# kestrelquantum/QuantumCollocation.jl

Hardware: AMD Instinct MI355X
Metric: full-trajectory constraint+Jacobian evals/s, 3-qubit T=1000 (higher is better)
Workload: dtype f64; 1 GPU; 3-qubit Toffoli UnitarySmoothPulseProblem, T=1000; T=1000 knots (1000/GPU), Pade order 4, free dt; T=1000, N=8, n_drives=6, kernel=mfma, parallelism=knot-shard x1, output_ring_buffers=17

## Files before the change

### quantumcollocation.jl_amd/csrc/qc_mfma_kernels.hip

```cpp
#include "qc_mfma_common.h"

namespace {

using namespace qc_mfma;

constexpr int kIntervalsPerWG = 1;
constexpr int kThreads = 128 * kIntervalsPerWG;
constexpr int kMaxGrid = 1024;

__device__ inline v4d load_GA(const double* __restrict__ Gx, int mat, int lane) { return load_image_tile(Gx + mat * 256, lane); }

constexpr int kDF = QC_DWIN_MAX_DERIV;


template <int kMU>
__device__ inline void request_images(int m, const double* __restrict__ Gx, int lane, v4d& g0, v4d (&gk)[kMU]) {
    g0 = load_GA(Gx, 0, lane);
#pragma unroll
    for (int u = 0; u < kMU; ++u) {
        const int k = u < m ? u : (m > 0 ? m - 1 : 0);
        gk[u] = load_GA(Gx, m > 0 ? k + 1 : 0, lane);
    }
}
template <int kMU>
__device__ inline void assemble_G_request(const QcParams& P, const double* __restrict__ Gx, const double* __restrict__ z0, int lane,
                                          v4d& g0, v4d (&gk)[kMU], double& av) {
    av = load_amp_lanes(z0, P.off_a, P.m, lane);
    request_images(P.m, Gx, lane, g0, gk);
}
template <int kMU>
__device__ inline v4d assemble_G_combine(const QcParams& P, const double* __restrict__ Gx, int lane, const v4d& g0, const v4d (&gk)[kMU],
                                         double av, double (&ak)[kMU]) {
    const int m = P.m;
    v4d Ga = g0;
#pragma unroll
    for (int u = 0; u < kMU; ++u) {
        ak[u] = (u < m) ? bcast_lane(av, u) : 0.0;
        Ga += ak[u] * gk[u];
    }
    for (int k = kMU; k < m; ++k) Ga += bcast_lane(av, k) * load_GA(Gx, k + 1, lane);
    return Ga;
}
template <int kMU>
__device__ inline v4d assemble_G(const QcParams& P, const double* __restrict__ Gx, const double* __restrict__ z0,
                                 int lane, v4d (&gk)[kMU], double (&ak)[kMU]) {
    v4d g0;
    double av;
    assemble_G_request(P, Gx, z0, lane, g0, gk, av);
    return assemble_G_combine(P, Gx, lane, g0, gk, av, ak);
}

template <int MODE>
__device__ inline void store_tile_T(double* __restrict__ p, const v4d& x, int g, int j) {
#pragma unroll
    for (int r = 0; r < 4; ++r) qc_st8m<MODE>(p + (4 * r + g) * 16 + j, x[r]);
}

template <int MODE>
__device__ inline void store_tile_T_masked(double* __restrict__ p, const v4d& x, int nr, int g, int j) {
#pragma unroll
    for (int r = 0; r < 4; ++r) if (4 * r + g < nr && j < nr) qc_st8m<MODE>(p + (4 * r + g) * nr + j, x[r]);
}
template <bool MASK>
__device__ inline v4d load_state_tile(const double* __restrict__ zU, int col, int nr, int g) {
    if constexpr (!MASK) {
        const double* p = zU + col * 16 + g;
        return v4d{p[0], p[4], p[8], p[12]};
    } else {
        const double* p = zU + col * nr;
        v4d v;
#pragma unroll
        for (int r = 0; r < 4; ++r) v[r] = (4 * r + g < nr) ? p[4 * r + g] : 0.0;
        return v;
    }
}

constexpr int kLdsGa = 0, kLdsU0 = 256, kLdsU1 = 512, kLdsGk = 768;

__device__ inline void lds_put(double* __restrict__ base, int lane, const v4d& x) {
    v2d* p = reinterpret_cast<v2d*>(base) + lane;
    p[0] = v2d{x[0], x[1]};
    p[64] = v2d{x[2], x[3]};
}
__device__ inline v4d lds_get(const double* __restrict__ base, int lane) {
    const v2d* p = reinterpret_cast<const v2d*>(base) + lane;
    const v2d lo = p[0], hi = p[64];
    return v4d{lo[0], lo[1], hi[0], hi[1]};
}
__device__ inline v2d load_knot128(const double* __restrict__ p, int lane) {
    typedef v2d __attribute__((aligned(8))) v2d_u;
    return reinterpret_cast<const v2d_u*>(p)[lane];
}
__device__ inline v4d lds_state_tile(const double* __restrict__ U, int col, int g) {
    const double* p = U + col * 16 + g;
    return v4d{p[0], p[4], p[8], p[12]};
}

#define QC_HOT_ARGS(P) (P).Gx, dZ, (P).t_begin, (P).n_int, (P).zdim, (P).off_a, (P).off_dt, (P).m

template <bool JAC, int MODE, bool DIAG, int kMU, bool KET, bool BATCH, bool ONCE = false, bool HEAD = false>
__global__ __launch_bounds__(JAC ? kThreads : 64, 2) void qc_mfma16_pade4_kernel(const double* __restrict__ hot_Gx, const double* __restrict__ Z, long long hot_t_begin, int hot_n_int,
                                                                      int hot_zdim, int hot_off_a, int hot_off_dt, int hot_m, const QcParams Pk,
                                                                      double* __restrict__ F, double* __restrict__ J,
                                                                      const QcParams* __restrict__ Pb) {
    const QcParams& P = BATCH ? Pb[blockIdx.y] : Pk;
    const int h_n_int = BATCH ? P.n_int : hot_n_int, h_zdim = BATCH ? P.zdim : hot_zdim, h_off_a = BATCH ? P.off_a : hot_off_a;
    const int h_off_dt = BATCH ? P.off_dt : hot_off_dt;
    const long long h_t_begin = BATCH ? P.t_begin : hot_t_begin;
    constexpr int kLdsD0 = kLdsGk + kMU * 256, kLdsD1 = kLdsD0 + 128;
    constexpr int kLdsBlock = kLdsD1 + 128;
    static_assert((kMU / 2 + 1) * 272 <= kLdsD0, "the windows must lie beyond the compute wave's transpose scratch");
    __shared__ __attribute__((aligned(16))) double sm_all[JAC ? kIntervalsPerWG * kLdsBlock : 2];
    unsigned long long t_entry = 0, t_kernarg = 0;
    if constexpr (DIAG) {
        t_entry = __builtin_amdgcn_s_memrealtime();
        const long long dep = (long long)Pk.N + Pk.n_deriv + Pk.drow[7] + Pk.jac_nnz + Pk.jo_d + Pk.ho_d + (long long)Pk.G + (long long)Pk.stamps +
                              (long long)Z + (long long)Pb + (long long)(Pk.c[2] != 0.0) + (long long)(Pk.dt_fixed != 0.0);
        asm volatile("s_memrealtime %0" : "=s"(t_kernarg) : "s"(dep));
    }
#ifndef QC_NO_KERNARG_TOUCH
    QcKernargTouch<sizeof(QcParams) + 96> touch;
    touch.request();
#endif
    const int tid = threadIdx.x;
    const int lane0 = tid & 63;
    const int wave = JAC ? __builtin_amdgcn_readfirstlane(tid >> 6) : 0;
    const int role = JAC ? 1 - wave / kIntervalsPerWG : 0;
    const int slot = wave % kIntervalsPerWG;
    double* __restrict__ sm = sm_all + (JAC ? slot * kLdsBlock : 0);
    const int ipw = JAC ? kIntervalsPerWG : 1;
    const int n_wg = (h_n_int + ipw - 1) / ipw;
    static_assert(!HEAD || (JAC && ONCE && !KET && !BATCH), "HEAD is a form of the loop-free unitary F + dF instantiation");
    const int m = HEAD ? kMU : BATCH ? P.m : hot_m;
    const int nc = KET ? P.nc : 8;
    const int nr = KET ? P.n : 16;
    const bool ft = HEAD || h_off_dt >= 0;
    const double c1 = P.c[1], c2 = P.c[2];
    const double* __restrict__ Gx = BATCH ? P.Gx : hot_Gx;

    v4d g0_img, gk_img[kMU];
    if (JAC && role == 1) request_images(m, Gx, lane0, g0_img, gk_img);
#ifndef QC_NO_KERNARG_TOUCH
    touch.consume();
#endif
    int vb = blockIdx.x;
    if (vb >= n_wg) return;
    do {
        int lane = lane0;
        if constexpr (!ONCE) asm volatile("" : "+v"(lane));
        const int g = lane >> 4, j = lane & 15, jj = j & 7;
        const int jc = (!KET || jj < nc) ? jj : 0;
        const bool left = j < 8;
        const v4d IdB = identity_B(g, j);
        const int b_raw = qc_xcd_remap(vb, n_wg) * ipw + slot;
        const bool active = b_raw < h_n_int;
        const int b = active ? b_raw : h_n_int - 1;
        const long long t = h_t_begin + b;
        const double* __restrict__ z0 = Z + t * (long long)h_zdim;
        const double* __restrict__ z1 = z0 + h_zdim;
        const double av_pre = (JAC && role == 1) ? load_amp_lanes(z0, h_off_a, m, lane) : 0.0;
        const double h_pre = ft ? load_uniform(z0 + h_off_dt) : opaque_scalar(P.dt_fixed);
        double* __restrict__ Jb = JAC ? J + (size_t)b * P.J_stride + P.J_off : nullptr;
        double* __restrict__ Fb = (HEAD || F) ? F + (size_t)b * P.F_stride + P.F_off : nullptr;
        QC_STAMP_DECL;

        if (HEAD ? __builtin_expect(role == 1, 1) : (JAC && role == 1)) {
            if (!active) { __syncthreads(); if constexpr (!ONCE) __syncthreads(); continue; }
            __builtin_amdgcn_s_setprio(3);
            if constexpr (DIAG) {
                qc_ts_[9] = t_entry;
                if (!(P.dbg_skip & 4)) { qc_ts_[10] = t_kernarg; qc_ts_[11] = __builtin_amdgcn_s_getreg((4 << 0) | (0 << 6) | (31 << 11)) | (1ull << 40); }
            }
            QC_STAMP(P, b, lane, 0);
            const double h = h_pre;
            double ak[kMU];
            const double av = av_pre;
            const v4d& g0 = g0_img;
            const v4d (&gk)[kMU] = gk_img;
            v4d u0, u1;
            v2d w_u0, w_u1;
            if constexpr (KET) {
                u0 = load_state_tile<true>(z0 + P.off_U, jc, nr, g);
                u1 = load_state_tile<true>(z1 + P.off_U, jc, nr, g);
            } else {
                w_u0 = load_knot128(z0 + P.off_U, lane);
                w_u1 = load_knot128(z1 + P.off_U, lane);
            }
            const int wo = P.dwin_lo + (2 * lane < P.dwin_n ? 2 * lane : 0);
            const v2d w_d0 = load_knot128(z0 + wo, 0), w_d1 = load_knot128(z1 + wo, 0);
            if (DIAG && (P.dbg_skip & 4)) {
                asm volatile("s_waitcnt lgkmcnt(0)" ::: "memory");
                QC_STAMP(P, b, lane, 10);
                asm volatile("s_waitcnt vmcnt(0)" ::: "memory");
                QC_STAMP(P, b, lane, 11);
            }
            v4d Ga;
            if constexpr (HEAD) {
                Ga = g0;
#pragma unroll
                for (int u = 0; u < kMU; ++u) Ga += bcast_lane(av, u) * gk[u];
            } else {
                Ga = assemble_G_combine(P, Gx, lane, g0, gk, av, ak);
            }
            const double hc1 = h * c1, hc2 = h * h * c2;
            QC_STAMP(P, b, lane, 1);
            bool skip = false;
            if constexpr (DIAG) skip = (P.dbg_skip & 1) != 0;
            const v4d Gb = mm16(Ga, IdB);
            const v4d G2T = mm16(Gb, Ga);
            v4d Fm, Bm;
#pragma unroll
            for (int r = 0; r < 4; ++r) {
                const double ev = IdB[r] + hc2 * G2T[r];
                Fm[r] = -(ev + hc1 * Ga[r]);
                Bm[r] = ev - hc1 * Ga[r];
            }
#ifndef QC_EARLY_COPIES
#define QC_EARLY_COPIES 4
#endif
            constexpr int kEarly = (!KET && ONCE) ? QC_EARLY_COPIES : 0;
            auto early_copy = [&](int q) {
                store_tile_T<MODE>(Jb + P.jo_F + q * 256, Fm, g, j);
                store_tile_T<MODE>(Jb + P.jo_B + q * 256, Bm, g, j);
            };
            auto hand_off = [&]() {
                lds_put(sm + kLdsGa, lane, Ga);
                if constexpr (KET) {
                    lds_put(sm + kLdsU0, lane, u0);
                    lds_put(sm + kLdsU1, lane, u1);
                } else {
                    reinterpret_cast<v2d*>(sm + kLdsU0)[lane] = w_u0;
                    reinterpret_cast<v2d*>(sm + kLdsU1)[lane] = w_u1;
                }
                reinterpret_cast<v2d*>(sm + kLdsD0)[lane] = w_d0;
                reinterpret_cast<v2d*>(sm + kLdsD1)[lane] = w_d1;
#pragma unroll
                for (int u = 0; u < kMU; ++u)
                    if (u < m) lds_put(sm + kLdsGk + u * 256, lane, gk[u]);
            };
            if constexpr (kEarly > 0) {
                if (HEAD || (!skip && P.copies >= kEarly)) {
#pragma unroll
                    for (int q = 0; q < kEarly; ++q) early_copy(q);
                    hand_off();
                } else {
                    if (!skip)
                        for (int q = 0; q < P.copies; ++q) early_copy(q);
                    hand_off();
                }
            } else {
                hand_off();
            }
            __syncthreads();
            if (!skip) {
                double* pF = Jb + P.jo_F;
                double* pB = Jb + P.jo_B;
                const int ncop = HEAD ? 8 : P.copies;
                for (int q = kEarly; q < ncop; ++q) {
                    if constexpr (!KET) {
                        store_tile_T<MODE>(pF + q * 256, Fm, g, j);
                        store_tile_T<MODE>(pB + q * 256, Bm, g, j);
                    } else {
                        store_tile_T_masked<MODE>(pF + q * nr * nr, Fm, nr, g, j);
                        store_tile_T_masked<MODE>(pB + q * nr * nr, Bm, nr, g, j);
                    }
                }
                __builtin_amdgcn_s_setprio(0);
                QC_STAMP(P, b, lane, 2);
                {
                    if (HEAD || P.dwin_n > 0) {
                        const double* w0 = sm + kLdsD0 - P.dwin_lo;
                        const double* w1 = sm + kLdsD1 - P.dwin_lo;
                        int jo = P.jo_d;
#pragma unroll
                        for (int d = 0; d < kDF; ++d) {
                            if (d < P.n_deriv) {
                                const int dim = P.ddim_i[d], r0 = P.drow[d];
                                if (lane < dim) {
                                    const double dxv = w0[P.dx_off[d] + lane];
                                    const double dfv = w1[P.x_off[d] + lane] - w0[P.x_off[d] + lane];
                                    if (Fb) Fb[r0 + lane] = dfv - h * dxv;
                                    Jb[jo + lane] = -1.0;
                                    Jb[jo + dim + lane] = 1.0;
                                    Jb[jo + 2 * dim + lane] = -h;
                                    if (ft) Jb[jo + 3 * dim + lane] = -dxv;
                                }
                                jo += (ft ? 4 : 3) * dim;
                            }
                        }
                    } else {
                        deriv_rows_generic(P, z0, z1, h, Fb, Jb, lane, false);
                    }
                }
                if constexpr (DIAG) {
                    asm volatile("s_waitcnt vmcnt(0)" ::: "memory");
                    QC_STAMP(P, b, lane, 3);
                }
                QC_STAMP_FLUSH(P, b, lane, 0, 3);
                QC_STAMP_FLUSH(P, b, lane, 9, 11);
            }
            if constexpr (!ONCE) __syncthreads();
            continue;
        }

        if (!active) { if constexpr (JAC) { __syncthreads(); if constexpr (!ONCE) __syncthreads(); } continue; }
        __builtin_amdgcn_s_setprio(1);
        QC_STAMP(P, b, lane, 4);
        QC_STAMP_CYCLES(13);
        const double h = h_pre;
        v4d u0, u1, Ga;
        v4d gk[kMU];
        if constexpr (JAC) {
            __syncthreads();
            Ga = lds_get(sm + kLdsGa, lane);
            if constexpr (KET) {
                u0 = lds_get(sm + kLdsU0, lane);
                u1 = lds_get(sm + kLdsU1, lane);
            } else {
                u0 = lds_state_tile(sm + kLdsU0, jc, g);
                u1 = lds_state_tile(sm + kLdsU1, jc, g);
            }
        } else {
            u0 = load_state_tile<KET>(z0 + P.off_U, jc, nr, g);
            u1 = load_state_tile<KET>(z1 + P.off_U, jc, nr, g);
            double ak[kMU];
            Ga = assemble_G(P, Gx, z0, lane, gk, ak);
        }
        const double hc1 = h * c1, hc2 = h * h * c2;
        QC_STAMP(P, b, lane, 5);
        bool skipc = false;
        if constexpr (DIAG) skipc = (P.dbg_skip & 2) != 0;
        if (!skipc) {
            v4d W, Wsw;
#pragma unroll
            for (int r = 0; r < 4; ++r) {
                const double sm_ = u1[r] + u0[r], df = u1[r] - u0[r];
                W[r] = left ? sm_ : df;
                Wsw[r] = left ? df : sm_;
            }
            const v4d P1 = mm16(Ga, W);
            const v4d P1sw = swap8(P1);
            v4d Q;
#pragma unroll
            for (int r = 0; r < 4; ++r) Q[r] = left ? (-hc1 * W[r] + hc2 * P1sw[r]) : (hc2 * W[r]);
            constexpr int NB = JAC ? kMU + 1 : 1;
            v4d sB[NB];
            {
                v4d aB[NB], bB[NB];
                aB[0] = Ga;
                bB[0] = P1sw;
                if constexpr (JAC) {
#pragma unroll
                    for (int u = 0; u < kMU; ++u) {
                        aB[u + 1] = lds_get(sm + kLdsGk + (u < m ? u : m - 1) * 256, lane);
                        bB[u + 1] = Q;
                    }
                }
                mm16_multi<NB>(aB, bB, sB);
            }
            const v4d P2 = sB[0];
            QC_STAMP(P, b, lane, 6);
            v4d E;
            {
                v4d dl, dh;
                const double d1 = -c1, d2 = 2.0 * c2 * h;
#pragma unroll
                for (int r = 0; r < 4; ++r) {
                    dl[r] = Wsw[r] - hc1 * P1[r] + hc2 * P2[r];
                    dh[r] = d1 * P1[r] + d2 * P2[r];
                }
                const v4d dhs = swap8(dh);
#pragma unroll
                for (int r = 0; r < 4; ++r) E[r] = left ? dl[r] : dhs[r];
            }
            constexpr int NC = JAC ? kMU / 2 + 1 : 1;
            v4d sC[NC];
            v4d Y[NC];
            {
                v4d aC[NC], bC[NC];
                aC[0] = E;
                bC[0] = IdB;
                if constexpr (JAC) {
#pragma unroll
                    for (int p2 = 0; p2 < kMU / 2; ++p2) {
                        const v4d R1 = sB[2 * p2 + 1], R2 = sB[2 * p2 + 2];
                        const v4d R1sw = swap8(R1), R2sw = swap8(R2);
                        aC[p2 + 1] = Ga;
#pragma unroll
                        for (int r = 0; r < 4; ++r) {
                            bC[p2 + 1][r] = left ? R1sw[r] : R2[r];
                            Y[p2 + 1][r] = left ? R1[r] : R2sw[r];
                        }
                    }
                }
                if constexpr (JAC) {
                    if constexpr (kMU / 2 > 0) {
                        v4d aT[kMU / 2], bT[kMU / 2], dT[kMU / 2];
#pragma unroll
                        for (int p2 = 0; p2 < kMU / 2; ++p2) { aT[p2] = aC[p2 + 1]; bT[p2] = bC[p2 + 1]; }
                        mm16_multi<kMU / 2>(aT, bT, dT);
#pragma unroll
                        for (int p2 = 0; p2 < kMU / 2; ++p2) sC[p2 + 1] = dT[p2];
                    }
                } else {
                    mm16_multi<NC>(aC, bC, sC);
                }
            }
            v4d ET;
            v4d YT[kMU / 2 > 0 ? kMU / 2 : 1];
            if constexpr (JAC) {
                v4d tin[kMU / 2 + 1], tout[kMU / 2 + 1];
                tin[0] = E;
#pragma unroll
                for (int p2 = 0; p2 < kMU / 2; ++p2) tin[p2 + 1] = Y[p2 + 1] + sC[p2 + 1];
                lds_transpose16_multi<kMU / 2 + 1>(sm, tin, tout, g, j);
                ET = tout[0];
#pragma unroll
                for (int p2 = 0; p2 < kMU / 2; ++p2) YT[p2] = tout[p2 + 1];
            } else {
                ET = sC[0];
            }
            auto store_ET = [&]() {
#pragma unroll
                for (int r = 0; r < 4; ++r) {
                    const int c = 4 * r + g;
                    if (c < 8) {
                        if (Fb && (!KET || (c < nc && j < nr))) qc_st8m<MODE>(Fb + c * nr + j, ET[r]);
                    } else if (JAC && ft && (!KET || (c - 8 < nc && j < nr))) {
                        qc_st8m<MODE>(Jb + P.jo_h + (c - 8) * nr + j, ET[r]);
                    }
                }
            };
            QC_STAMP(P, b, lane, 7);
            if constexpr (!JAC) {
                store_ET();
                deriv_rows_generic(P, z0, z1, h, Fb, nullptr, lane, false);
            } else {
                double* pa = Jb + P.jo_a;
                auto store_pair = [&](int k, const v4d& YTk) {
                    const bool two = k + 1 < m;
                    const int sk = KET ? P.s : 128;
                    double* p = pa + (size_t)k * sk;
#pragma unroll
                    for (int r = 0; r < 4; ++r) {
                        const int c = 4 * r + g;
                        if (r < 2) { if (!KET || (c < nc && j < nr)) qc_st8m<MODE>(p + c * nr + j, YTk[r]); }
                        else if (two && (!KET || (c - 8 < nc && j < nr))) qc_st8m<MODE>(p + sk + (c - 8) * nr + j, YTk[r]);
                    }
                };
                QC_STAMP(P, b, lane, 8);
                store_ET();
#pragma unroll
                for (int u = 0; u < kMU; u += 2)
                    if (u < m) store_pair(u, YT[u >> 1]);
                for (int k = kMU; k < m; k += 2) {
                    const v4d R1 = mm16(load_GA(Gx, k + 1, lane), Q);
                    const v4d R2 = mm16(load_GA(Gx, k + 2 <= m ? k + 2 : k + 1, lane), Q);
                    const v4d R1sw = swap8(R1), R2sw = swap8(R2);
                    v4d X, Yk;
#pragma unroll
                    for (int r = 0; r < 4; ++r) {
                        X[r] = left ? R1sw[r] : R2[r];
                        Yk[r] = left ? R1[r] : R2sw[r];
                    }
                    Yk += mm16(Ga, X);
                    store_pair(k, mm16(Yk, IdB));
                }
            }
            if constexpr (DIAG) {
                asm volatile("s_waitcnt vmcnt(0)" ::: "memory");
                QC_STAMP(P, b, lane, 12);
                QC_STAMP_CYCLES(14);
            }
            if constexpr (DIAG) qc_ts_[15] = __builtin_amdgcn_s_getreg((4 << 0) | (0 << 6) | (31 << 11)) | (1ull << 40);
            QC_STAMP_FLUSH(P, b, lane, 4, 8);
            QC_STAMP_FLUSH(P, b, lane, 12, 15);
        }
        if constexpr (JAC && !ONCE) __syncthreads();
    } while (!ONCE && (vb += gridDim.x) < n_wg);
}

}

bool qc_mfma_pade4_supported(const QcParams& P) {
    return P.integrator == QC_PADE && P.p == 2 && ((P.n <= 16 && P.nc <= 8) || (P.n <= 32 && P.nc <= 16)) && P.m <= 32;
}

size_t qc_mfma_gx_doubles(const QcParams& P) {
    if (P.n > 32) return qc_mfma64_gx_doubles(P);
    return P.n > 16 ? qc_mfma32_gx_doubles(P) : (size_t)2 * (P.m + 1) * 256;
}

void qc_mfma_pack_G(const QcParams& P, const double* G, double* Gx) {
    if (P.n > 32) { qc_mfma64_pack_G(P, G, Gx); return; }
    if (P.n > 16) { qc_mfma32_pack_G(P, G, Gx); return; }
    const int n = P.n, M = P.m + 1;
    for (int mat = 0; mat < M; ++mat) {
        const double* A = G + (size_t)mat * n * n;
        for (int pr = 0; pr < 2; ++pr)
            for (int l = 0; l < 64; ++l)
                for (int e = 0; e < 2; ++e) {
                    const int g = l >> 4, i = l & 15, kk = 2 * pr + e, c = 4 * kk + g;
                    const bool in = i < n && c < n;
                    Gx[((size_t)mat * 2 + pr) * 128 + l * 2 + e] = in ? A[(size_t)c * n + i] : 0.0;
                    Gx[((size_t)(M + mat) * 2 + pr) * 128 + l * 2 + e] = in ? A[(size_t)i * n + c] : 0.0;
                }
    }
}

template <bool JAC, bool DIAG, int MU>
static void launch16m(const QcParams& P, const double* dZ, double* dF, double* dJ, hipStream_t st, int grid, int threads) {
    if (P.nc != 8 || P.n != 16) {
        const int n_wg_k = JAC ? (P.n_int + kIntervalsPerWG - 1) / kIntervalsPerWG : P.n_int;
        if (grid == n_wg_k) hipLaunchKernelGGL((qc_mfma16_pade4_kernel<JAC, 2, false, MU, true, false, true>), dim3(grid), dim3(threads), 0, st, QC_HOT_ARGS(P), P, dF, dJ, nullptr);
        else hipLaunchKernelGGL((qc_mfma16_pade4_kernel<JAC, 2, false, MU, true, false>), dim3(grid), dim3(threads), 0, st, QC_HOT_ARGS(P), P, dF, dJ, nullptr);
        return;
    }
    const int n_wg = JAC ? (P.n_int + kIntervalsPerWG - 1) / kIntervalsPerWG : P.n_int;
    switch (P.store_mode) {
        case 0: hipLaunchKernelGGL((qc_mfma16_pade4_kernel<JAC, 0, DIAG, MU, false, false>), dim3(grid), dim3(threads), 0, st, QC_HOT_ARGS(P), P, dF, dJ, nullptr); break;
        case 1: hipLaunchKernelGGL((qc_mfma16_pade4_kernel<JAC, 1, DIAG, MU, false, false>), dim3(grid), dim3(threads), 0, st, QC_HOT_ARGS(P), P, dF, dJ, nullptr); break;
        default:
            if constexpr (JAC) {
                if (grid == n_wg && P.head && P.dbg_skip == 0 && P.m == MU && P.copies == 8 && P.copies >= QC_EARLY_COPIES && P.dwin_n > 0 && P.off_dt >= 0 && dF != nullptr && P.antisym) {
                    hipLaunchKernelGGL((qc_mfma16_pade4_kernel<JAC, 2, DIAG, MU, false, false, true, true>), dim3(grid), dim3(threads), 0, st, QC_HOT_ARGS(P), P, dF, dJ, nullptr);
                    break;
                }
            }
            if (grid == n_wg)
                hipLaunchKernelGGL((qc_mfma16_pade4_kernel<JAC, 2, DIAG, MU, false, false, true>), dim3(grid), dim3(threads), 0, st, QC_HOT_ARGS(P), P, dF, dJ, nullptr);
            else
                hipLaunchKernelGGL((qc_mfma16_pade4_kernel<JAC, 2, DIAG, MU, false, false>), dim3(grid), dim3(threads), 0, st, QC_HOT_ARGS(P), P, dF, dJ, nullptr);
            break;
    }
}

template <bool JAC, bool DIAG>
static void launch16(const QcParams& P, const double* dZ, double* dF, double* dJ, hipStream_t st, int grid, int threads) {
    if (P.m <= 2) launch16m<JAC, DIAG, 2>(P, dZ, dF, dJ, st, grid, threads);
    else if (P.m <= 4) launch16m<JAC, DIAG, 4>(P, dZ, dF, dJ, st, grid, threads);
    else if (P.m <= 6) launch16m<JAC, DIAG, 6>(P, dZ, dF, dJ, st, grid, threads);
    else launch16m<JAC, DIAG, 8>(P, dZ, dF, dJ, st, grid, threads);
}

bool qc_mfma16_batchable(const QcParams& P, const QcClass& cls) {
    return P.integrator == QC_PADE && P.p == 2 && P.n <= 16 && P.nc <= 8 && P.m <= 32 && P.store_mode == 2 && !cls.stamped && P.dbg_skip == 0;
}

template <bool JAC, int MU>
static void launch16_batch(const QcParams& P0, const QcParams* dPb, int count, const double* dZ, double* dF, double* dJ, hipStream_t st, int grid,
                           int threads) {
    if (P0.nc != 8 || P0.n != 16)
        hipLaunchKernelGGL((qc_mfma16_pade4_kernel<JAC, 2, false, MU, true, true>), dim3(grid, count), dim3(threads), 0, st, QC_HOT_ARGS(P0), P0, dF, dJ, dPb);
    else
        hipLaunchKernelGGL((qc_mfma16_pade4_kernel<JAC, 2, false, MU, false, true>), dim3(grid, count), dim3(threads), 0, st, QC_HOT_ARGS(P0), P0, dF, dJ, dPb);
}

hipError_t qc_launch_mfma16_F_jac_batch(const QcParams& P0, const QcParams* dPb, int count, const double* dZ, double* dF, double* dJ,
                                        hipStream_t st) {
    const int n_wg = dJ ? (P0.n_int + kIntervalsPerWG - 1) / kIntervalsPerWG : P0.n_int;
    const int grid = n_wg < kMaxGrid ? n_wg : kMaxGrid;
    const int threads = dJ ? kThreads : 64;
#define QC_B(J_, MU_) launch16_batch<J_, MU_>(P0, dPb, count, dZ, dF, dJ, st, grid, threads)
    if (dJ) { if (P0.m <= 2) QC_B(true, 2); else if (P0.m <= 4) QC_B(true, 4); else if (P0.m <= 6) QC_B(true, 6); else QC_B(true, 8); }
    else    { if (P0.m <= 2) QC_B(false, 2); else if (P0.m <= 4) QC_B(false, 4); else if (P0.m <= 6) QC_B(false, 6); else QC_B(false, 8); }
#undef QC_B
    return hipGetLastError();
}

hipError_t qc_launch_mfma16_F_jac(const QcParams& P, const double* dZ, double* dF, double* dJ, hipStream_t st) {
    const int n_wg = dJ ? (P.n_int + kIntervalsPerWG - 1) / kIntervalsPerWG : P.n_int;
    const int grid = n_wg < kMaxGrid ? n_wg : kMaxGrid;
    const bool diag = P.stamps != nullptr || P.dbg_skip != 0;
    if (dJ) { if (diag) launch16<true, true>(P, dZ, dF, dJ, st, grid, kThreads); else launch16<true, false>(P, dZ, dF, dJ, st, grid, kThreads); }
    else    { if (diag) launch16<false, true>(P, dZ, dF, dJ, st, grid, 64); else launch16<false, false>(P, dZ, dF, dJ, st, grid, 64); }
    return hipGetLastError();
}
```

Before: 124,400 evals/s (T=1000-equivalent).

## Stage F-only unitary knot state and derivative window through LDS with coalesced loads

For the F-only, non-ket, non-batched, single-pass kernel variant, the two knots' unitary state and derivative-variable windows are fetched with wide coalesced 128-element loads, written to LDS, and read back as MFMA tiles after a wavefront barrier. The derivative constraint rows are then computed from the LDS window instead of the generic global-memory path. Generator images and control amplitudes are also prefetched early, as the Jacobian path already does. This adds LDS use and a barrier, and it only affects the constraint-only evaluation path. A Python script is included that compares the generated assembly.

```diff
diff --git a/profiles/ipopt_forms_asm_diff.py b/profiles/ipopt_forms_asm_diff.py
--- /dev/null
+++ b/profiles/ipopt_forms_asm_diff.py
@@ -0,0 +1,66 @@
+#!/usr/bin/env python3
+import argparse
+import os
+import re
+import subprocess
+import sys
+
+from sweep_asm_diff import KEYS, relabel, show
+
+FILES = {"qc_mfma_kernels": 8, "qc_mfma_hess_g2": 2}
+REWRITTEN = re.compile(r"qc_mfma16_pade4_kernel<false, 2, (?:false|true), \d, false, false, true, false>")
+
+
+def kernels(path, n_args):
+    txt = open(path).read()
+    notes = txt[txt.rfind("amdhsa.kernels"):]
+    out = {}
+    for m in re.finditer(r"^(_Z\w+):\s*; @\1\n(.*?)^\.Lfunc_end\d+:", txt, re.S | re.M):
+        name = m.group(1)
+        k = re.search(r"\.amdhsa_kernel %s\n(.*?)\.end_amdhsa_kernel" % name, txt, re.S)
+        if not k:
+            continue
+        body = [re.sub(r"\s*;.*$", "", ln) for ln in relabel(m.group(2)).replace(name, "KERNEL").splitlines()]
+        body = [ln for ln in body if ln.strip()]
+        blk = [b for b in re.split(r"\n  - \.agpr_count", notes) if re.search(r"\.name:\s+%s\n" % name, b)]
+        assert len(blk) == 1, name
+        meta = {key: int(re.search(r"\.%s:\s+(\d+)" % key, ".agpr_count" + blk[0]).group(1)) for key in KEYS}
+        meta["instructions"] = sum(1 for ln in body if ln.startswith("\t") and not ln.strip().startswith("."))
+        out[plain(name, n_args)] = ("\n".join(body), relabel(k.group(1)).replace(name, "KERNEL"), meta)
+    return out
+
+
+def plain(name, n_args):
+    o = subprocess.run(["c++filt", name], capture_output=True, text=True).stdout.strip().replace("(anonymous namespace)::", "")
+    base, args = re.match(r"(?:void )?([\w:]+)<([^>]*)>", o).groups()
+    args = [re.sub(r"^\(\w+\)", "", x.strip()) for x in args.split(",")]
+    return "%s<%s>" % (base, ", ".join(args + ["false"] * (n_args - len(args))))
+
+
+def main():
+    ap = argparse.ArgumentParser()
+    ap.add_argument("parent")
+    ap.add_argument("new")
+    a = ap.parse_args()
+    differ = same = 0
+    report = []
+    for f, n_args in FILES.items():
+        A, B = (kernels(os.path.join(d, f + ".s"), n_args) for d in (a.parent, a.new))
+        for p in sorted(set(A) | set(B)):
+            if REWRITTEN.fullmatch(p) or (p in B and p not in A):
+                for label, K in (("parent", A), ("new   ", B)):
+                    if p in K:
+                        report.append(f"{p}  {label}: {show(K[p][2])}")
+            elif p in A and p in B and A[p] == B[p]:
+                same += 1
+            else:
+                differ += 1
+                print(f"{f}.hip  {p}: DIFFERS" if p in B else f"{f}.hip  {p}: on the parent's side only")
+    print("\n".join(report))
+    print(f"{same} instantiations identical in instruction stream and metadata, {differ} differ or are gone "
+          f"(the rewritten and the new ones, listed above, not counted)")
+    return 1 if differ else 0
+
+
+if __name__ == "__main__":
+    sys.exit(main())
diff --git a/quantumcollocation.jl_amd/csrc/qc_mfma_kernels.hip b/quantumcollocation.jl_amd/csrc/qc_mfma_kernels.hip
--- a/quantumcollocation.jl_amd/csrc/qc_mfma_kernels.hip
+++ b/quantumcollocation.jl_amd/csrc/qc_mfma_kernels.hip
@@ -110,7 +110,9 @@
     constexpr int kLdsD0 = kLdsGk + kMU * 256, kLdsD1 = kLdsD0 + 128;
     constexpr int kLdsBlock = kLdsD1 + 128;
     static_assert((kMU / 2 + 1) * 272 <= kLdsD0, "the windows must lie beyond the compute wave's transpose scratch");
-    __shared__ __attribute__((aligned(16))) double sm_all[JAC ? kIntervalsPerWG * kLdsBlock : 2];
+    constexpr bool kFOnce = !JAC && MODE == 2 && !KET && !BATCH && ONCE;
+    constexpr int kLdsFU0 = 0, kLdsFU1 = 128, kLdsFD0 = 256, kLdsFD1 = 384;
+    __shared__ __attribute__((aligned(16))) double sm_all[JAC ? kIntervalsPerWG * kLdsBlock : (kFOnce ? 512 : 2)];
     unsigned long long t_entry = 0, t_kernarg = 0;
     if constexpr (DIAG) {
         t_entry = __builtin_amdgcn_s_memrealtime();
@@ -139,7 +141,7 @@
     const double* __restrict__ Gx = BATCH ? P.Gx : hot_Gx;
 
     v4d g0_img, gk_img[kMU];
-    if (JAC && role == 1) request_images(m, Gx, lane0, g0_img, gk_img);
+    if ((JAC && role == 1) || kFOnce) request_images(m, Gx, lane0, g0_img, gk_img);
 #ifndef QC_NO_KERNARG_TOUCH
     touch.consume();
 #endif
@@ -158,7 +160,7 @@
         const long long t = h_t_begin + b;
         const double* __restrict__ z0 = Z + t * (long long)h_zdim;
         const double* __restrict__ z1 = z0 + h_zdim;
-        const double av_pre = (JAC && role == 1) ? load_amp_lanes(z0, h_off_a, m, lane) : 0.0;
+        const double av_pre = ((JAC && role == 1) || kFOnce) ? load_amp_lanes(z0, h_off_a, m, lane) : 0.0;
         const double h_pre = ft ? load_uniform(z0 + h_off_dt) : opaque_scalar(P.dt_fixed);
         double* __restrict__ Jb = JAC ? J + (size_t)b * P.J_stride + P.J_off : nullptr;
         double* __restrict__ Fb = (HEAD || F) ? F + (size_t)b * P.F_stride + P.F_off : nullptr;
@@ -320,6 +322,21 @@
                 u0 = lds_state_tile(sm + kLdsU0, jc, g);
                 u1 = lds_state_tile(sm + kLdsU1, jc, g);
             }
+        } else if constexpr (kFOnce) {
+            const v2d w_u0 = load_knot128(z0 + P.off_U, lane), w_u1 = load_knot128(z1 + P.off_U, lane);
+            const int wo = P.dwin_lo + (2 * lane < P.dwin_n ? 2 * lane : 0);
+            const v2d w_d0 = load_knot128(z0 + wo, 0), w_d1 = load_knot128(z1 + wo, 0);
+            double ak[kMU];
+            Ga = assemble_G_combine(P, Gx, lane, g0_img, gk_img, av_pre, ak);
+            reinterpret_cast<v2d*>(sm + kLdsFU0)[lane] = w_u0;
+            reinterpret_cast<v2d*>(sm + kLdsFU1)[lane] = w_u1;
+            reinterpret_cast<v2d*>(sm + kLdsFD0)[lane] = w_d0;
+            reinterpret_cast<v2d*>(sm + kLdsFD1)[lane] = w_d1;
+            __builtin_amdgcn_fence(__ATOMIC_RELEASE, "wavefront");
+            __builtin_amdgcn_wave_barrier();
+            __builtin_amdgcn_fence(__ATOMIC_ACQUIRE, "wavefront");
+            u0 = lds_state_tile(sm + kLdsFU0, jc, g);
+            u1 = lds_state_tile(sm + kLdsFU1, jc, g);
         } else {
             u0 = load_state_tile<KET>(z0 + P.off_U, jc, nr, g);
             u1 = load_state_tile<KET>(z1 + P.off_U, jc, nr, g);
@@ -434,7 +451,25 @@
             QC_STAMP(P, b, lane, 7);
             if constexpr (!JAC) {
                 store_ET();
-                deriv_rows_generic(P, z0, z1, h, Fb, nullptr, lane, false);
+                if (kFOnce && P.dwin_n > 0) {
+                    if (Fb) {
+                        const double* w0 = sm + kLdsFD0 - P.dwin_lo;
+                        const double* w1 = sm + kLdsFD1 - P.dwin_lo;
+#pragma unroll
+                        for (int d = 0; d < kDF; ++d) {
+                            if (d < P.n_deriv) {
+                                const int dim = P.ddim_i[d], r0 = P.drow[d];
+                                if (lane < dim) {
+                                    const double dxv = w0[P.dx_off[d] + lane];
+                                    const double dfv = w1[P.x_off[d] + lane] - w0[P.x_off[d] + lane];
+                                    Fb[r0 + lane] = dfv - h * dxv;
+                                }
+                            }
+                        }
+                    }
+                } else {
+                    deriv_rows_generic(P, z0, z1, h, Fb, nullptr, lane, false);
+                }
             } else {
                 double* pa = Jb + P.jo_a;
                 auto store_pair = [&](int k, const v4d& YTk) {
```

Result: no change. 123,600 evals/s (T=1000-equivalent) (-0.6%).
